# arnab39/equiadapt

Hardware: AMD Instinct MI355X
Metric: canonicalize+invert images/sec (224x224 C8) (higher is better)
Workload: dtype f32 (resampling / FFT / accumulation in fp32; the network's channel contraction as 2xfp16 split of every fp32 operand (within one fp32 ulp), 3 exact products, fp32 accumulate -- closer to fp64 than the fp32 matrix instruction, see step_ms_by_gemm_form); 1 GPU; configs[1]: 224x224x3 synthetic, C8, GroupEquivariantImageCanonicalization + ESCNNEquivariantNetwork in e2cnn's LAYER SHAPES (32 fields x 8 = 256 ch, k5, 3 layers, crop 0.8, resize 96) with this repository's own filter-bank parameterisation (bilinear-rotated banks; e2cnn's steerable basis is not restated -- e2cnn-trained weights enter via load_exported_dense), forward, then invert_canonicalization; batch_per_gpu=256, global_batch=256, parallelism=dp1 (no collective in the forward path)

## Files before the change

### equiadapt_amd/csrc/cgemm3m_bf16.hip

```cpp
#include "eqa_common.hpp"

#ifdef EQA_BLK_CLOCK
namespace {
__device__ long long g_blk_clock[16];
struct BlkClock {
  long long c0, w0, e0, t_epi;
  unsigned long long tk[8], tot[8];
  __device__ __forceinline__ BlkClock() : c0(clock64()), w0(wall_clock64()), e0(0), t_epi(0), tk{}, tot{} {}
  __device__ __forceinline__ void tick(int i) {
    if constexpr (EQA_BLK_CLOCK >= 2) {
      __builtin_amdgcn_sched_barrier(0);
      asm volatile("s_memtime %0" : "=s"(tk[i]));
    }
  }
  __device__ __forceinline__ void stage_end() {
    if constexpr (EQA_BLK_CLOCK >= 2) {
      tick(5);
      asm volatile("s_waitcnt lgkmcnt(0)" ::: "memory");
#pragma unroll
      for (int i = 0; i < 5; ++i) tot[i] += tk[i + 1] - tk[i];
    }
  }
  __device__ __forceinline__ void tile_epilogue_begin() { e0 = clock64(); }
  __device__ __forceinline__ void tile_epilogue_end() { t_epi += clock64() - e0; }
  __device__ __forceinline__ void publish() {
    if (blockIdx.x == 100 && threadIdx.x == 0) {
      g_blk_clock[0] = clock64() - c0; g_blk_clock[1] = wall_clock64() - w0; g_blk_clock[2] = t_epi;
      for (int i = 0; i < 7; ++i) g_blk_clock[3 + i] = (long long)tot[i];
    }
  }
};
}
extern "C" int eqa_debug_blk_clock(long long* out) { return (int)hipMemcpyFromSymbol(out, HIP_SYMBOL(g_blk_clock), 80); }
#else
namespace {
struct BlkClock {
  __device__ __forceinline__ void tick(int) {}
  __device__ __forceinline__ void stage_end() {}
  __device__ __forceinline__ void tile_epilogue_begin() {}
  __device__ __forceinline__ void tile_epilogue_end() {}
  __device__ __forceinline__ void publish() {}
};
}
#endif

namespace {

#include "cgemm3m_common.inc"

typedef __bf16 bf16x8 __attribute__((ext_vector_type(8)));
typedef unsigned u32x2 __attribute__((ext_vector_type(2)));

constexpr unsigned kHi = 0xffff0000u;

__device__ __forceinline__ void split3(const float a, unsigned (&x)[3]) {
  const float p1 = __builtin_bit_cast(float, __builtin_bit_cast(unsigned, a) & kHi);
  const float r1 = a - p1;
  const float p2 = __builtin_bit_cast(float, __builtin_bit_cast(unsigned, r1) & kHi);
  const float r2 = r1 - p2;
  x[0] = __builtin_bit_cast(unsigned, a);
  x[1] = __builtin_bit_cast(unsigned, r1);
  x[2] = __builtin_bit_cast(unsigned, r2);
}
__device__ __forceinline__ unsigned pack_hi(const unsigned lo, const unsigned hi) { return __builtin_amdgcn_perm(hi, lo, 0x07060302u); }

struct Pieces {
  u32x4 p[3];
};
__device__ __forceinline__ Pieces split8(const f32x4 lo, const f32x4 hi) {
  Pieces o;
  unsigned x[8][3];
#pragma unroll
  for (int e = 0; e < 8; ++e) split3(e < 4 ? lo[e & 3] : hi[e & 3], x[e]);
#pragma unroll
  for (int j = 0; j < 4; ++j)
#pragma unroll
    for (int q = 0; q < 3; ++q) o.p[q][j] = pack_hi(x[2 * j][q], x[2 * j + 1][q]);
  return o;
}
__device__ __forceinline__ void split4(const f32x4 v, u32x2 (&o)[3]) {
  unsigned x[4][3];
#pragma unroll
  for (int t = 0; t < 4; ++t) split3(v[t], x[t]);
#pragma unroll
  for (int q = 0; q < 3; ++q) {
    o[q][0] = pack_hi(x[0][q], x[1][q]);
    o[q][1] = pack_hi(x[2][q], x[3][q]);
  }
}

struct ARaw {
  f32x4 ar[2], ai[2];
};
struct BHalf {
  u32x4 b[3][3];
};
struct APieces {
  Pieces a[2][3];
};

constexpr unsigned kBFrag = 64 * 16;
constexpr unsigned kBTileBytes = 9 * kBFrag;

__device__ __forceinline__ void load_a(ARaw& o, const StageAddr& at, unsigned aoff) {
#pragma unroll
  for (int b = 0; b < 2; ++b) {
    o.ar[b] = buf_ld<f32x4>(at.a, aoff + 32 * b, at.sa);
    o.ai[b] = buf_ld<f32x4>(at.a, aoff + 32 * b + 64, at.sa);
  }
}
__device__ __forceinline__ void load_b(BHalf& o, const StageAddr& at, unsigned boff, int n) {
#pragma unroll
  for (int p = 0; p < 3; ++p)
#pragma unroll
    for (int q = 0; q < 3; ++q) o.b[p][q] = buf_ld<u32x4>(at.b, boff + ((n * 3 + p) * 3 + q) * kBFrag, at.sb);
}

__device__ __forceinline__ void split_a(APieces& P, const ARaw& r, int m) {
  P.a[m][0] = split8(r.ar[0], r.ar[1]);
  P.a[m][1] = split8(r.ai[0], r.ai[1]);
  P.a[m][2] = split8(r.ar[0] + r.ai[0], r.ar[1] + r.ai[1]);
}

__device__ __forceinline__ f32x16 mma(const u32x4 a, const u32x4 b, const f32x16 c) {
  return __builtin_amdgcn_mfma_f32_32x32x16_bf16(__builtin_bit_cast(bf16x8, a), __builtin_bit_cast(bf16x8, b), c, 0, 0, 0);
}

template <int TERMS>
__device__ __forceinline__ void mma_quarter(const APieces& P, const BHalf& B, f32x16 (&acc)[3][2][2], int m, int n) {
#pragma unroll
  for (int w = 0; w < 5; ++w)
#pragma unroll
    for (int pa = 0; pa < 3; ++pa) {
      const int pb = w - pa;
      if (pb < 0 || pb > 2 || (TERMS == 6 && w > 2)) continue;
#pragma unroll
      for (int p = 0; p < 3; ++p) acc[p][m][n] = mma(P.a[m][p].p[pa], B.b[p][pb], acc[p][m][n]);
    }
}

template <int NMMA, int NVALU, int NLOAD, int NSTORE, int NDS>
__device__ __forceinline__ void pin_quarter() {
  if (NDS) __builtin_amdgcn_sched_group_barrier(0x100, NDS, 0);
  constexpr int kMem = NLOAD + NSTORE;
  constexpr int kValuPer = (NVALU + NMMA - 1) / NMMA;
#pragma unroll
  for (int k = 0; k < NMMA; ++k) {
    __builtin_amdgcn_sched_group_barrier(0x008, 1, 0);
    if (k < NLOAD) __builtin_amdgcn_sched_group_barrier(0x020, 1, 0);
    else if (k < kMem) __builtin_amdgcn_sched_group_barrier(0x040, 1, 0);
    if (NVALU) __builtin_amdgcn_sched_group_barrier(0x002, kValuPer, 0);
  }
}

template <int NPAIR, int TERMS>
__device__ __forceinline__ void run_stage(APieces& P, ARaw& raw0, ARaw& raw1, BHalf& B0, BHalf& B1, f32x16 (&acc)[3][2][2],
                                          const StageAddr& cur, const StageAddr& nxt, unsigned naoff0, unsigned naoff1, unsigned boff,
                                          const float* lds_lane, const ParkedDst& dst, int p0) {
  constexpr int kQ = 3 * TERMS;
  constexpr int kSplit = 150;
  f32x4 park[NPAIR > 0 ? NPAIR : 1];
  __builtin_amdgcn_sched_barrier(0);
  load_b(B1, cur, boff, 1);
  load_a(raw0, nxt, naoff0);
  split_a(P, raw1, 1);
  mma_quarter<TERMS>(P, B0, acc, 0, 0);
  pin_quarter<kQ, kSplit, 13, 0, 0>();
  __builtin_amdgcn_sched_barrier(0);
  load_a(raw1, nxt, naoff1);
  mma_quarter<TERMS>(P, B0, acc, 1, 0);
  pin_quarter<kQ, 0, 4, 0, 0>();
  __builtin_amdgcn_sched_barrier(0);
#pragma unroll
  for (int k = 0; k < NPAIR; ++k) park[k] = *reinterpret_cast<const f32x4*>(lds_lane + (p0 + k) * (2 * kLdsRowFloats));
  load_b(B0, nxt, boff, 0);
  mma_quarter<TERMS>(P, B1, acc, 0, 1);
#pragma unroll
  for (int k = 0; k < NPAIR; ++k) store_pair(dst, p0 + k, park[k]);
  pin_quarter<kQ, 0, 9, NPAIR, NPAIR>();
  __builtin_amdgcn_sched_barrier(0);
  split_a(P, raw0, 0);
  mma_quarter<TERMS>(P, B1, acc, 1, 1);
  pin_quarter<kQ, kSplit, 0, 0, 0>();
  __builtin_amdgcn_sched_barrier(0);
}

template <int NPAIR, int TERMS>
__global__ __launch_bounds__(256, 1) void fft_cgemm3m_bf16_kernel(const float* __restrict__ V, const uint16_t* __restrict__ Bp,
                                                                  float* __restrict__ Mo, int M, int pitch, int Cin, int Cout, int F,
                                                                  int n_rt, int n_ct, int waves_per_xcd) {
  const int lane = threadIdx.x & 63;
  const int wave = __builtin_amdgcn_readfirstlane(threadIdx.x >> 6);
  const int xcd = blockIdx.x & (kXcd - 1);
  const int q = (blockIdx.x >> 3) * 4 + wave;
  const int S = Cin / kStageK;
  const int wpf = n_rt * n_ct;
  const int nf_x = (F - xcd + kXcd - 1) / kXcd;
  const int total = nf_x * wpf;
  if (q >= total) return;
  const int i = lane & 31, h = lane >> 5;
  __shared__ __attribute__((aligned(16))) float lds_all[4 * kLdsWaveFloats];
  float* lds_w = lds_all + wave * kLdsWaveFloats;
  const float* lds_lane = lds_w + h * kLdsRowFloats + i * 4;
  const WaveTileWalk<uint16_t, kBTileBytes> walk(V, Bp, Mo, M, pitch, Cin, Cout, xcd, wpf, n_ct, S, i, h);
  const unsigned boff = lane * 16;

  StageAddr at;
  unsigned aoff0, aoff1;
  int f, row0, ct;
  walk.locate(q, at, aoff0, aoff1, f, row0, ct);
  ParkedDst dst = walk.nothing_parked(f, row0, ct);
  ARaw raw0, raw1;
  APieces P;
  BHalf B0, B1;
  load_a(raw0, at, aoff0);
  load_a(raw1, at, aoff1);
  load_b(B0, at, boff, 0);
  split_a(P, raw0, 0);
  for (int u = q; u < total; u += waves_per_xcd) {
    f32x16 acc[3][2][2];
#pragma unroll
    for (int p = 0; p < 3; ++p)
#pragma unroll
      for (int m = 0; m < 2; ++m)
#pragma unroll
        for (int n = 0; n < 2; ++n)
#pragma unroll
          for (int e = 0; e < 16; ++e) acc[p][m][n][e] = 0.f;
    StageAddr nat;
    unsigned naoff0, naoff1;
    int nf, nrow0, nct;
    walk.locate(u + waves_per_xcd < total ? u + waves_per_xcd : u, nat, naoff0, naoff1, nf, nrow0, nct);
    for (int s = 0; s < S; ++s) {
      const bool more = s + 1 < S;
      if (NPAIR == 0) flush_rows(lds_lane, dst, (32 * s) / S, (32 * (s + 1)) / S);
      run_stage<NPAIR, TERMS>(P, raw0, raw1, B0, B1, acc, walk.at_stage(at, s), more ? walk.at_stage(at, s + 1) : nat,
                              more ? aoff0 : naoff0, more ? aoff1 : naoff1, boff, lds_lane, dst, s * NPAIR);
    }
    park_tile(acc, lds_w, i, h);
    dst = walk.parked(f, row0, ct);
    at = nat; aoff0 = naoff0; aoff1 = naoff1; f = nf; row0 = nrow0; ct = nct;
  }
  flush_rows(lds_lane, dst, 0, 32);
}

constexpr int kBlkM = 128, kBlkN = 128;
constexpr int kFragBytes = 64 * 16;
constexpr int kABufs = 3;
typedef _Float16 f16x8 __attribute__((ext_vector_type(8)));

constexpr int pieces_of(int terms) { return terms == 3 ? 2 : 3; }
constexpr int a_stage_bytes(int terms) { return 12 * pieces_of(terms) * kFragBytes; }

template <int NP>
struct BSet {
  u32x4 b[3][NP];
};
struct AFrags {
  u32x4 a[3];
};
struct RawA {
  f32x4 re[2], im[2];
};
struct TileAt {
  __amdgpu_buffer_rsrc_t a, b;
  unsigned sb;
};

typedef _Float16 f16x2v __attribute__((ext_vector_type(2)));
__device__ __forceinline__ void split4h(const f32x4 v, u32x2 (&o)[2]) {
#pragma unroll
  for (int j = 0; j < 2; ++j) {
    const float a = v[2 * j], b = v[2 * j + 1];
    const f16x2v h = {(_Float16)a, (_Float16)b};
    const f16x2v l = {(_Float16)(a - (float)h[0]), (_Float16)(b - (float)h[1])};
    o[0][j] = __builtin_bit_cast(unsigned, h);
    o[1][j] = __builtin_bit_cast(unsigned, l);
  }
}
template <int NP, int ROW, int PART>
__device__ __forceinline__ void split_part(const RawA& r, unsigned char* wr, const float scale) {
  const f32x4 v = PART == 0 ? r.re[ROW] : PART == 1 ? r.im[ROW] : r.re[ROW] + r.im[ROW];
  u32x2 o[NP];
  if constexpr (NP == 3) split4(v, o);
  else split4h(v * scale, o);
#pragma unroll
  for (int q = 0; q < NP; ++q) *reinterpret_cast<u32x2*>(wr + (ROW * 6 * NP + PART * NP + q) * kFragBytes) = o[q];
}
template <int ROW>
__device__ __forceinline__ void load_raw(RawA& o, const TileAt& t, unsigned voff, unsigned row64, unsigned soff) {
  o.re[ROW] = buf_ld<f32x4>(t.a, voff + ROW * row64, soff);
  o.im[ROW] = buf_ld<f32x4>(t.a, voff + ROW * row64 + 64, soff);
}
template <int NP>
__device__ __forceinline__ void load_bset(BSet<NP>& o, const TileAt& t, unsigned voff, unsigned soff) {
#pragma unroll
  for (int k = 0; k < 3 * NP; ++k) o.b[k / NP][k % NP] = buf_ld<u32x4>(t.b, voff + k * kBFrag, t.sb + soff);
}
template <int NP, int M, int PA>
__device__ __forceinline__ void read_frags(AFrags& o, const unsigned char* rd) {
#pragma unroll
  for (int p = 0; p < 3; ++p) o.a[p] = *reinterpret_cast<const u32x4*>(rd + ((M * 3 + p) * NP + PA) * kFragBytes);
}
template <int TERMS>
__device__ __forceinline__ f32x16 mma_t(const u32x4 a, const u32x4 b, const f32x16 c) {
  if constexpr (TERMS == 3) return __builtin_amdgcn_mfma_f32_32x32x16_f16(__builtin_bit_cast(f16x8, a), __builtin_bit_cast(f16x8, b), c, 0, 0, 0);
  else return mma(a, b, c);
}
template <int TERMS, int M, int PA, bool FIRST>
__device__ __forceinline__ void mma_rows(const AFrags& A, const BSet<pieces_of(TERMS)>& B, f32x16 (&acc)[3][4]) {
  const f32x16 zero = {0.f, 0.f, 0.f, 0.f, 0.f, 0.f, 0.f, 0.f, 0.f, 0.f, 0.f, 0.f, 0.f, 0.f, 0.f, 0.f};
#pragma unroll
  for (int pb = 0; pb < pieces_of(TERMS); ++pb) {
    if ((TERMS == 6 && PA + pb > 2) || (TERMS == 3 && PA + pb > 1)) continue;
#pragma unroll
    for (int p = 0; p < 3; ++p) acc[p][M] = mma_t<TERMS>(A.a[p], B.b[p][pb], FIRST && PA == 0 && pb == 0 ? zero : acc[p][M]);
  }
}
template <int NMMA, int NDSR, int NLOAD, int NVALU, int NDSW>
__device__ __forceinline__ void pin_region() {
  constexpr int kValuPer = (NVALU + NMMA - 1) / NMMA;
#pragma unroll
  for (int k = 0; k < NMMA; ++k) {
    __builtin_amdgcn_sched_group_barrier(0x008, 1, 0);
    if (k < NDSR) __builtin_amdgcn_sched_group_barrier(0x100, 1, 0);
    if (k < NLOAD) __builtin_amdgcn_sched_group_barrier(0x020, 1, 0);
    if (NVALU) __builtin_amdgcn_sched_group_barrier(0x002, kValuPer, 0);
    if (k >= NMMA - NDSW) __builtin_amdgcn_sched_group_barrier(0x200, 1, 0);
  }
}

template <int TERMS, bool FIRST>
__device__ __forceinline__ void run_stage_block(const BSet<pieces_of(TERMS)>& Bc, BSet<pieces_of(TERMS)>& Bn, RawA& raw, AFrags& F0,
                                                AFrags& F1, AFrags& F2, AFrags& F3,
                                                f32x16 (&acc)[3][4], const unsigned char* rd, const unsigned char* rd_next,
                                                unsigned char* wr, const TileAt& tb, unsigned sb_off, unsigned b_voff, const TileAt& ta,
                                                unsigned sa_off, unsigned a_voff, unsigned row64, const float scale, BlkClock& clk) {
  constexpr int NP = pieces_of(TERMS);
  constexpr int kN = TERMS == 9 ? 27 : TERMS == 6 ? 18 : 9;
  constexpr int kSplit = NP == 3 ? 32 : 20;
  constexpr int kRd = 3 * NP;
  clk.tick(0);
  __builtin_amdgcn_sched_barrier(0);
  read_frags<NP, 0, 1>(F1, rd);
  if constexpr (NP == 3) read_frags<NP, 0, 2>(F2, rd);
  read_frags<NP, 1, 0>(F3, rd);
  load_bset<NP>(Bn, tb, b_voff, sb_off);
  split_part<NP, 0, 0>(raw, wr, scale);
  mma_rows<TERMS, 0, 0, FIRST>(F0, Bc, acc); mma_rows<TERMS, 0, 1, FIRST>(F1, Bc, acc);
  if constexpr (NP == 3) mma_rows<TERMS, 0, 2, FIRST>(F2, Bc, acc);
  pin_region<kN, kRd, kRd, kSplit, NP>();
  clk.tick(1);
  __builtin_amdgcn_sched_barrier(0);
  read_frags<NP, 1, 1>(F1, rd);
  if constexpr (NP == 3) read_frags<NP, 1, 2>(F2, rd);
  read_frags<NP, 2, 0>(F0, rd);
  split_part<NP, 0, 1>(raw, wr, scale); split_part<NP, 0, 2>(raw, wr, scale);
  mma_rows<TERMS, 1, 0, FIRST>(F3, Bc, acc); mma_rows<TERMS, 1, 1, FIRST>(F1, Bc, acc);
  if constexpr (NP == 3) mma_rows<TERMS, 1, 2, FIRST>(F2, Bc, acc);
  pin_region<kN, kRd, 0, 2 * kSplit + 4, 2 * NP>();
  clk.tick(2);
  __builtin_amdgcn_sched_barrier(0);
  read_frags<NP, 2, 1>(F1, rd);
  if constexpr (NP == 3) read_frags<NP, 2, 2>(F2, rd);
  read_frags<NP, 3, 0>(F3, rd);
  split_part<NP, 1, 0>(raw, wr, scale); split_part<NP, 1, 1>(raw, wr, scale);
  mma_rows<TERMS, 2, 0, FIRST>(F0, Bc, acc); mma_rows<TERMS, 2, 1, FIRST>(F1, Bc, acc);
  if constexpr (NP == 3) mma_rows<TERMS, 2, 2, FIRST>(F2, Bc, acc);
  pin_region<kN, kRd, 0, 2 * kSplit, 2 * NP>();
  clk.tick(3);
  __builtin_amdgcn_sched_barrier(0);
  read_frags<NP, 3, 1>(F1, rd);
  if constexpr (NP == 3) read_frags<NP, 3, 2>(F2, rd);
  read_frags<NP, 0, 0>(F0, rd_next);
  split_part<NP, 1, 2>(raw, wr, scale);
  load_raw<0>(raw, ta, a_voff, row64, sa_off);
  mma_rows<TERMS, 3, 0, FIRST>(F3, Bc, acc); mma_rows<TERMS, 3, 1, FIRST>(F1, Bc, acc);
  if constexpr (NP == 3) mma_rows<TERMS, 3, 2, FIRST>(F2, Bc, acc);
  pin_region<kN, kRd, 2, kSplit + 4, NP>();
  __builtin_amdgcn_sched_barrier(0);
  load_raw<1>(raw, ta, a_voff, row64, sa_off);
  clk.tick(4);
  __builtin_amdgcn_sched_barrier(0);
  asm volatile("s_waitcnt lgkmcnt(0)\n\ts_barrier" ::: "memory");
  clk.stage_end();
}

template <int TERMS>
__global__ __launch_bounds__(256, 1) void fft_cgemm3m_bf16_block_kernel(const float* __restrict__ V, const uint16_t* __restrict__ Bp,
                                                                        float* __restrict__ Mo, int M, int pitch, int Cin, int Cout, int F,
                                                                        int n_rt, int n_cg, int blocks_per_xcd,
                                                                        const float* __restrict__ vbound, int nbound, float b_scale) {
  constexpr int NP = pieces_of(TERMS);
  constexpr int kAStageBytes = a_stage_bytes(TERMS);
  const int lane = threadIdx.x & 63;
  const int wave = __builtin_amdgcn_readfirstlane(threadIdx.x >> 6);
  const int xcd = blockIdx.x & (kXcd - 1);
  const int q = blockIdx.x >> 3;
  const int S = Cin / kStageK;
  const int tpf = n_rt * n_cg;
  const int nf_x = (F - xcd + kXcd - 1) / kXcd;
  const int total = nf_x * tpf;
  if (q >= total) return;
  BlkClock clk;
  extern __shared__ __attribute__((aligned(16))) unsigned char lds[];
  const size_t rowf = (size_t)2 * Cin, mo_row = (size_t)2 * Cout;
  const unsigned b_stage_bytes = (unsigned)(Cout / 32) * 3 * NP * kBFrag;
  const unsigned a_stage = 32u * 4u;
  const unsigned b_voff = lane * 16;
  const unsigned row64 = (unsigned)(64 * rowf * 4);
  const int sp_b = lane & 1, sp_r = (lane >> 1) & 15, sp_h = lane >> 5;
  const int sp_row = 16 * wave + sp_r;
  const unsigned sp_lds = (unsigned)((sp_row >> 5) * 3 * NP * kFragBytes + ((sp_row & 31) + 32 * sp_h) * 16 + 8 * sp_b);
  const unsigned sp_k = (unsigned)(8 * sp_b + 4 * sp_h) * 4u;

  auto locate = [&](int u, TileAt& at, unsigned& aoff, int& f, int& row0, int& ct) {
    const bool live = u < total;
    const int uu = live ? u : 0;
    const int fi = uu / tpf, r = uu - fi * tpf;
    f = xcd + kXcd * fi;
    const int rt = r / n_cg, cg = r - rt * n_cg;
    row0 = rt * kBlkM;
    ct = 4 * cg + wave;
    at.a = __builtin_amdgcn_make_buffer_rsrc(const_cast<float*>(V) + (size_t)f * pitch * rowf, 0, live ? (unsigned)((size_t)pitch * rowf * 4) : 0u, 0x00020000);
    aoff = (unsigned)((size_t)(row0 + sp_row) * rowf * 4) + sp_k;
    at.b = __builtin_amdgcn_make_buffer_rsrc(const_cast<uint16_t*>(Bp) + (size_t)f * S * (b_stage_bytes / 2), 0, live ? (unsigned)S * b_stage_bytes : 0u, 0x00020000);
    at.sb = (unsigned)ct * (3 * NP * kBFrag);
  };

  TileAt ta, tb;
  unsigned a_voff, b_unused;
  int ua = q, sa = 0, ub = q, sb = 0;
  int fa, rowa, cta, f, row0, ct;
  locate(q, ta, a_voff, f, row0, ct);
  tb = ta;
  auto next_a = [&]() {
    if (++sa == S) { sa = 0; ua += blocks_per_xcd; locate(ua, ta, a_voff, fa, rowa, cta); }
  };
  auto next_b = [&]() {
    if (++sb == S) { sb = 0; ub += blocks_per_xcd; locate(ub, tb, b_unused, fa, rowa, cta); }
  };

  float a_scale = 1.0f, out_scale = 1.0f;
  if constexpr (TERMS == 3) {
    float mx = 0.0f;
    for (int t = lane; t < nbound; t += 64) mx = fmaxf(mx, vbound[t]);
#pragma unroll
    for (int o = 32; o > 0; o >>= 1) mx = fmaxf(mx, __shfl_xor(mx, o));
    int ex = 0;
    if (mx > 0.0f && mx < 3.0e38f) (void)frexpf(mx, &ex);
    ex = min(max(14 - ex, -100), 100);
    ex = __builtin_amdgcn_readfirstlane(ex);
    a_scale = ldexpf(1.0f, ex);
    out_scale = ldexpf(1.0f, -ex) / b_scale;
  }
  RawA raw0, raw1;
  BSet<NP> B0, B1;
  AFrags F0, F1, F2, F3;
  load_raw<0>(raw0, ta, a_voff, row64, sa * a_stage); load_raw<1>(raw0, ta, a_voff, row64, sa * a_stage); next_a();
  load_raw<0>(raw1, ta, a_voff, row64, sa * a_stage); load_raw<1>(raw1, ta, a_voff, row64, sa * a_stage); next_a();
  load_bset<NP>(B0, tb, b_voff, sb * b_stage_bytes); next_b();
  {
    unsigned char* w0p = lds + sp_lds;
    unsigned char* w1p = lds + kAStageBytes + sp_lds;
    split_part<NP, 0, 0>(raw0, w0p, a_scale); split_part<NP, 0, 1>(raw0, w0p, a_scale); split_part<NP, 0, 2>(raw0, w0p, a_scale);
    split_part<NP, 1, 0>(raw0, w0p, a_scale); split_part<NP, 1, 1>(raw0, w0p, a_scale); split_part<NP, 1, 2>(raw0, w0p, a_scale);
    split_part<NP, 0, 0>(raw1, w1p, a_scale); split_part<NP, 0, 1>(raw1, w1p, a_scale); split_part<NP, 0, 2>(raw1, w1p, a_scale);
    split_part<NP, 1, 0>(raw1, w1p, a_scale); split_part<NP, 1, 1>(raw1, w1p, a_scale); split_part<NP, 1, 2>(raw1, w1p, a_scale);
  }
  load_raw<0>(raw0, ta, a_voff, row64, sa * a_stage); load_raw<1>(raw0, ta, a_voff, row64, sa * a_stage); next_a();
  load_raw<0>(raw1, ta, a_voff, row64, sa * a_stage); load_raw<1>(raw1, ta, a_voff, row64, sa * a_stage); next_a();
  asm volatile("s_waitcnt lgkmcnt(0)\n\ts_barrier" ::: "memory");
  unsigned rbuf = 0;
  read_frags<NP, 0, 0>(F0, lds + lane * 16);
  auto step = [&](unsigned o) { return o + kAStageBytes >= kABufs * kAStageBytes ? o + kAStageBytes - kABufs * kAStageBytes : o + kAStageBytes; };

  for (int u = q; u < total; u += blocks_per_xcd) {
    f32x16 acc[3][4];
#define EQA_STAGE(FIRST, BC, BN, RAW)                                                                                                 \
  {                                                                                                                                  \
    const unsigned r1 = step(rbuf), r2 = step(r1);                                                                                   \
    run_stage_block<TERMS, FIRST>(BC, BN, RAW, F0, F1, F2, F3, acc, lds + rbuf + lane * 16, lds + r1 + lane * 16, lds + r2 + sp_lds, \
                                  tb, sb * b_stage_bytes, b_voff, ta, sa * a_stage, a_voff, row64, a_scale, clk);                            \
    next_a(); next_b();                                                                                                              \
    rbuf = r1;                                                                                                                       \
  }
    EQA_STAGE(true, B0, B1, raw0)
    EQA_STAGE(false, B1, B0, raw1)
    for (int s = 2; s < S; s += 2) {
      EQA_STAGE(false, B0, B1, raw0)
      EQA_STAGE(false, B1, B0, raw1)
    }
#undef EQA_STAGE
    clk.tile_epilogue_begin();
    {
      const int rows = __builtin_amdgcn_readfirstlane(min(kBlkM, M - row0));
      const __amdgpu_buffer_rsrc_t dr =
          __builtin_amdgcn_make_buffer_rsrc(Mo + ((size_t)f * pitch + row0) * mo_row, 0, (unsigned)(rows * mo_row * 4), 0x00020000);
      const int i = lane & 31, h = lane >> 5;
      const unsigned voff = (unsigned)((4 * h * mo_row + (size_t)(32 * ct + i) * 2) * 4);
#pragma unroll
      for (int m = 0; m < 4; ++m)
#pragma unroll
        for (int e = 0; e < 16; ++e) {
          const unsigned roff = voff + (unsigned)((32 * m + (e & 3) + 8 * (e >> 2)) * mo_row * 4);
          const float t1 = acc[0][m][e], t2 = acc[1][m][e], t3 = acc[2][m][e];
          u32x2 c;
          c[0] = __builtin_bit_cast(unsigned, TERMS == 3 ? (t1 - t2) * out_scale : t1 - t2);
          c[1] = __builtin_bit_cast(unsigned, TERMS == 3 ? (t3 - t1 - t2) * out_scale : t3 - t1 - t2);
          __builtin_amdgcn_raw_buffer_store_b64(c, dr, roff, 0, 0);
        }
    }
    int nf, nrow0, nct;
    TileAt unused_t;
    unsigned unused_o;
    locate(u + blocks_per_xcd, unused_t, unused_o, nf, nrow0, nct);
    f = nf; row0 = nrow0; ct = nct;
    clk.tile_epilogue_end();
  }
  clk.publish();
}

__global__ __launch_bounds__(256) void spectra3m_split_kernel(const float* __restrict__ B3, uint16_t* __restrict__ Bp, size_t groups) {
  const size_t t = (size_t)blockIdx.x * blockDim.x + threadIdx.x;
  if (t >= groups * 64) return;
  const size_t g = t >> 6;
  const int lane = (int)(t & 63);
  const float* src = B3 + g * (2 * 64 * 4) + lane * 4;
  const f32x4 lo = *reinterpret_cast<const f32x4*>(src), hi = *reinterpret_cast<const f32x4*>(src + 64 * 4);
  const Pieces p = split8(lo, hi);
  u32x4* dst = reinterpret_cast<u32x4*>(Bp + g * (3 * 64 * 8)) + lane;
#pragma unroll
  for (int q = 0; q < 3; ++q) dst[q * 64] = p.p[q];
}


__global__ __launch_bounds__(256) void spectra3m_split_f16_kernel(const float* __restrict__ B3, uint16_t* __restrict__ Bh, size_t groups,
                                                                  float b_scale) {
  const size_t t = (size_t)blockIdx.x * blockDim.x + threadIdx.x;
  if (t >= groups * 64) return;
  const size_t g = t >> 6;
  const int lane = (int)(t & 63);
  const float* src = B3 + g * (2 * 64 * 4) + lane * 4;
  const f32x4 lo = *reinterpret_cast<const f32x4*>(src) * b_scale, hi = *reinterpret_cast<const f32x4*>(src + 64 * 4) * b_scale;
  u32x2 a[2], b[2];
  split4h(lo, a);
  split4h(hi, b);
  u32x4* dst = reinterpret_cast<u32x4*>(Bh + g * (2 * 64 * 8)) + lane;
#pragma unroll
  for (int q = 0; q < 2; ++q) {
    const u32x4 v = {a[q][0], a[q][1], b[q][0], b[q][1]};
    dst[q * 64] = v;
  }
}

template <int TERMS>
int launch_block(const float* V, const void* B, float* Mo, int64_t M, int Cin, int Cout, const float* vbound, int nbound, float b_scale,
                 void* stream) {
  const int n_rb = (int)((M + kBlkM - 1) / kBlkM), n_cg = Cout / kBlkN;
  constexpr int kLds = kABufs * a_stage_bytes(TERMS);
  if (!allow_dynamic_lds((const void*)fft_cgemm3m_bf16_block_kernel<TERMS>, kLds)) return EQA_ERR_LAUNCH;
  hipLaunchKernelGGL((fft_cgemm3m_bf16_block_kernel<TERMS>), dim3(kGridBlocks), dim3(256), kLds, (hipStream_t)stream, V,
                     static_cast<const uint16_t*>(B), Mo, (int)M, (int)eqa_fft48k5_tile_pitch(M), Cin, Cout, eqa_fft48k5_frequencies(), n_rb,
                     n_cg, kBlocksPerXcd, vbound, nbound, b_scale);
  return launch_status();
}

}

namespace eqa {
int g_cgemm_bf16_form = 0;
}

extern "C" {

int64_t eqa_fft48k5_spectra3m_bf16_bytes(int Cin, int Cout) {
  if (!eqa_fft48k5_cgemm3m_supported(Cin, Cout)) return 0;
  return (int64_t)eqa_fft48k5_frequencies() * Cin * Cout * 3 * 3 * 2;
}

int eqa_fft48k5_spectra3m_split(const float* B3, void* Bp, int Cin, int Cout, void* stream) {
  if (!B3 || !Bp) return EQA_ERR_INVALID_ARG;
  if (!eqa_fft48k5_cgemm3m_supported(Cin, Cout) || (((uintptr_t)B3 | (uintptr_t)Bp) & 15)) return EQA_ERR_UNSUPPORTED;
  const size_t groups = (size_t)eqa_fft48k5_frequencies() * (Cin / kStageK) * (Cout / 32) * 3;
  const size_t threads = groups * 64;
  hipLaunchKernelGGL(spectra3m_split_kernel, dim3((unsigned)((threads + 255) / 256)), dim3(256), 0, (hipStream_t)stream, B3,
                     static_cast<uint16_t*>(Bp), groups);
  return launch_status();
}

int eqa_fft48k5_cgemm3m_bf16x3(const float* V, const void* Bp, float* Mo, int64_t M, int Cin, int Cout, int terms, void* stream) {
  if (terms != 9 && terms != 6) return EQA_ERR_INVALID_ARG;
  const int st = check_contraction_args(V, Bp, Mo, M, Cin, Cout);
  if (st != EQA_OK) return st == kNothingToDo ? EQA_OK : st;
  if ((int64_t)Cin * Cout * 9 * 2 > 0x7fffffffLL) return EQA_ERR_UNSUPPORTED;
  if (Cout % kBlkN == 0 && eqa::g_cgemm_bf16_form != 1) {
    return terms == 9 ? launch_block<9>(V, Bp, Mo, M, Cin, Cout, nullptr, 0, 1.0f, stream)
                      : launch_block<6>(V, Bp, Mo, M, Cin, Cout, nullptr, 0, 1.0f, stream);
  }
  const int F = eqa_fft48k5_frequencies();
  const int n_rt = (int)((M + kTileM - 1) / kTileM), n_ct = Cout / kTileN;
  const int S = Cin / kStageK;
#define EQA_CG_LAUNCH(NP, T)                                                                                                            \
  hipLaunchKernelGGL((fft_cgemm3m_bf16_kernel<NP, T>), dim3(kGridBlocks), dim3(256), 0, (hipStream_t)stream, V,                         \
                     static_cast<const uint16_t*>(Bp), Mo, (int)M, (int)eqa_fft48k5_tile_pitch(M), Cin, Cout, F, n_rt, n_ct, kWavesPerXcd)
#define EQA_CG_TERMS(NP) do { if (terms == 9) EQA_CG_LAUNCH(NP, 9); else EQA_CG_LAUNCH(NP, 6); } while (0)
  switch (32 % S == 0 ? 32 / S : 0) {
    case 4: EQA_CG_TERMS(4); break;
    case 2: EQA_CG_TERMS(2); break;
    case 1: EQA_CG_TERMS(1); break;
    default: EQA_CG_TERMS(0); break;
  }
#undef EQA_CG_TERMS
#undef EQA_CG_LAUNCH
  return launch_status();
}


int64_t eqa_fft48k5_spectra3m_f16_bytes(int Cin, int Cout) {
  if (!eqa_fft48k5_cgemm3m_supported(Cin, Cout) || Cout % kBlkN != 0) return 0;
  return (int64_t)eqa_fft48k5_frequencies() * Cin * Cout * 3 * 2 * 2;
}

int eqa_fft48k5_spectra3m_split_f16(const float* B3, void* Bh, int Cin, int Cout, float b_scale, void* stream) {
  if (!B3 || !Bh || !(b_scale > 0.0f)) return EQA_ERR_INVALID_ARG;
  if (eqa_fft48k5_spectra3m_f16_bytes(Cin, Cout) == 0 || (((uintptr_t)B3 | (uintptr_t)Bh) & 15)) return EQA_ERR_UNSUPPORTED;
  int ex = 0;
  if (frexpf(b_scale, &ex) != 0.5f) return EQA_ERR_INVALID_ARG;
  const size_t groups = (size_t)eqa_fft48k5_frequencies() * (Cin / kStageK) * (Cout / 32) * 3;
  const size_t threads = groups * 64;
  hipLaunchKernelGGL(spectra3m_split_f16_kernel, dim3((unsigned)((threads + 255) / 256)), dim3(256), 0, (hipStream_t)stream, B3,
                     static_cast<uint16_t*>(Bh), groups, b_scale);
  return launch_status();
}

int eqa_fft48k5_cgemm3m_f16x2(const float* V, const void* Bh, float* Mo, int64_t M, int Cin, int Cout, const float* vbound, int nbound,
                              float b_scale, void* stream) {
  if (!vbound || nbound <= 0 || !(b_scale > 0.0f)) return EQA_ERR_INVALID_ARG;
  const int st = check_contraction_args(V, Bh, Mo, M, Cin, Cout);
  if (st != EQA_OK) return st == kNothingToDo ? EQA_OK : st;
  if (Cout % kBlkN != 0 || (Cin / kStageK) % 2 != 0 || (int64_t)Cin * Cout * 6 * 2 > 0x7fffffffLL) return EQA_ERR_UNSUPPORTED;
  return launch_block<3>(V, Bh, Mo, M, Cin, Cout, vbound, nbound, b_scale, stream);
}

}
```

Before: 74840 images/s.

## Overlap tile epilogue stores with last K-stage matrix instructions

The final K-stage of each tile becomes a specialized LAST variant. Once an accumulator row block is final, its output stores are interleaved with the remaining matrix instructions of later row blocks, so only the last row block is written in the separate epilogue. This hides the serial store epilogue behind MFMA work. Stores also get a nontemporal cache hint, and the timing probe gains a last-stage counter. The cost is more complex scheduling pins and a restructured stage loop, which may disturb register pressure or instruction ordering.

```diff
diff --git a/equiadapt_amd/csrc/cgemm3m_bf16.hip b/equiadapt_amd/csrc/cgemm3m_bf16.hip
--- a/equiadapt_amd/csrc/cgemm3m_bf16.hip
+++ b/equiadapt_amd/csrc/cgemm3m_bf16.hip
@@ -4,9 +4,9 @@
 namespace {
 __device__ long long g_blk_clock[16];
 struct BlkClock {
-  long long c0, w0, e0, t_epi;
+  long long c0, w0, e0, t_epi, l0, t_last;
   unsigned long long tk[8], tot[8];
-  __device__ __forceinline__ BlkClock() : c0(clock64()), w0(wall_clock64()), e0(0), t_epi(0), tk{}, tot{} {}
+  __device__ __forceinline__ BlkClock() : c0(clock64()), w0(wall_clock64()), e0(0), t_epi(0), l0(0), t_last(0), tk{}, tot{} {}
   __device__ __forceinline__ void tick(int i) {
     if constexpr (EQA_BLK_CLOCK >= 2) {
       __builtin_amdgcn_sched_barrier(0);
@@ -21,12 +21,15 @@
       for (int i = 0; i < 5; ++i) tot[i] += tk[i + 1] - tk[i];
     }
   }
+  __device__ __forceinline__ void last_stage_begin() { l0 = clock64(); }
+  __device__ __forceinline__ void last_stage_end() { t_last += clock64() - l0; }
   __device__ __forceinline__ void tile_epilogue_begin() { e0 = clock64(); }
   __device__ __forceinline__ void tile_epilogue_end() { t_epi += clock64() - e0; }
   __device__ __forceinline__ void publish() {
     if (blockIdx.x == 100 && threadIdx.x == 0) {
       g_blk_clock[0] = clock64() - c0; g_blk_clock[1] = wall_clock64() - w0; g_blk_clock[2] = t_epi;
-      for (int i = 0; i < 7; ++i) g_blk_clock[3 + i] = (long long)tot[i];
+      for (int i = 0; i < 6; ++i) g_blk_clock[3 + i] = (long long)tot[i];
+      g_blk_clock[9] = t_last;
     }
   }
 };
@@ -37,6 +40,8 @@
 struct BlkClock {
   __device__ __forceinline__ void tick(int) {}
   __device__ __forceinline__ void stage_end() {}
+  __device__ __forceinline__ void last_stage_begin() {}
+  __device__ __forceinline__ void last_stage_end() {}
   __device__ __forceinline__ void tile_epilogue_begin() {}
   __device__ __forceinline__ void tile_epilogue_end() {}
   __device__ __forceinline__ void publish() {}
@@ -329,13 +334,101 @@
     if (k >= NMMA - NDSW) __builtin_amdgcn_sched_group_barrier(0x200, 1, 0);
   }
 }
-
-template <int TERMS, bool FIRST>
+template <int NMMA, int NDSR, int NLOAD, int NVALU, int NDSW>
+__device__ __forceinline__ void pin_region_head() {
+  constexpr int kValuPer = (NVALU + NMMA - 1) / NMMA, kRdPer = (NDSR + NMMA - 1) / NMMA;
+#pragma unroll
+  for (int k = 0; k < NMMA; ++k) {
+    __builtin_amdgcn_sched_group_barrier(0x008, 1, 0);
+    __builtin_amdgcn_sched_group_barrier(0x100, kRdPer, 0);
+    if (k < NLOAD) __builtin_amdgcn_sched_group_barrier(0x020, 1, 0);
+    __builtin_amdgcn_sched_group_barrier(0x002, kValuPer, 0);
+  }
+  __builtin_amdgcn_sched_group_barrier(0x200, NDSW, 0);
+}
+
+struct TileDst {
+  __amdgpu_buffer_rsrc_t dr;
+  unsigned voff, row_bytes;
+  float out_scale;
+};
+constexpr int kStoreNt = 2;
+template <int TERMS, int MQ, int E0 = 0, int E1 = 16>
+__device__ __forceinline__ void retire_rows(const f32x16 (&acc)[3][4], const TileDst& d) {
+#pragma unroll
+  for (int e = E0; e < E1; ++e) {
+    const unsigned roff = d.voff + (unsigned)(32 * MQ + (e & 3) + 8 * (e >> 2)) * d.row_bytes;
+    const float t1 = acc[0][MQ][e], t2 = acc[1][MQ][e], t3 = acc[2][MQ][e];
+    u32x2 c;
+    c[0] = __builtin_bit_cast(unsigned, TERMS == 3 ? (t1 - t2) * d.out_scale : t1 - t2);
+    c[1] = __builtin_bit_cast(unsigned, TERMS == 3 ? (t3 - t1 - t2) * d.out_scale : t3 - t1 - t2);
+    __builtin_amdgcn_raw_buffer_store_b64(c, d.dr, roff, 0, kStoreNt);
+  }
+}
+
+template <int TERMS>
+constexpr int mma_code(int k) {
+  int n = 0;
+  for (int pa = 0; pa < pieces_of(TERMS); ++pa)
+    for (int pb = 0; pb < pieces_of(TERMS); ++pb) {
+      if ((TERMS == 6 && pa + pb > 2) || (TERMS == 3 && pa + pb > 1)) continue;
+      for (int p = 0; p < 3; ++p)
+        if (n++ == k) return (pa * 3 + pb) * 3 + p;
+    }
+  return -1;
+}
+template <int TERMS, int M, int K>
+__device__ __forceinline__ void mma_one(const AFrags& Fa, const AFrags& Fb, const AFrags& Fc, const BSet<pieces_of(TERMS)>& B,
+                                        f32x16 (&acc)[3][4]) {
+  constexpr int code = mma_code<TERMS>(K), pa = code / 9, pb = code / 3 % 3, p = code % 3;
+  static_assert(code >= 0, "no such matrix instruction in a region");
+  const AFrags& A = pa == 0 ? Fa : pa == 1 ? Fb : Fc;
+  acc[p][M] = mma_t<TERMS>(A.a[p], B.b[p][pb], acc[p][M]);
+}
+template <int TERMS, int M, int K>
+__device__ __forceinline__ void retire_slot(const AFrags& Fa, const AFrags& Fb, const AFrags& Fc, const BSet<pieces_of(TERMS)>& B,
+                                            f32x16 (&acc)[3][4], const TileDst& d) {
+  constexpr int kN = 3 * (TERMS == 3 ? 3 : TERMS), kS = kN / 3, kR = kN - kS;
+  constexpr int kRet = TERMS == 3 ? 9 : 7;
+  constexpr int e0 = (K - kS) * 16 / kR, e1 = (K - kS + 1) * 16 / kR;
+  mma_one<TERMS, M, K>(Fa, Fb, Fc, B, acc);
+  retire_rows<TERMS, M - 1, e0, e1>(acc, d);
+  __builtin_amdgcn_sched_group_barrier(0x008, 1, 0);
+#pragma unroll
+  for (int e = e0; e < e1; ++e) {
+    __builtin_amdgcn_sched_group_barrier(0x002, kRet, 0);
+    __builtin_amdgcn_sched_group_barrier(0x040, 1, 0);
+  }
+  __builtin_amdgcn_sched_barrier(0);
+}
+template <int TERMS, int M, int K0, int... K>
+__device__ __forceinline__ void retire_slots(const AFrags& Fa, const AFrags& Fb, const AFrags& Fc, const BSet<pieces_of(TERMS)>& B,
+                                             f32x16 (&acc)[3][4], const TileDst& d, std::integer_sequence<int, K...>) {
+  (retire_slot<TERMS, M, K0 + K>(Fa, Fb, Fc, B, acc, d), ...);
+}
+template <int TERMS, int M, int... K>
+__device__ __forceinline__ void mma_head(const AFrags& Fa, const AFrags& Fb, const AFrags& Fc, const BSet<pieces_of(TERMS)>& B,
+                                         f32x16 (&acc)[3][4], std::integer_sequence<int, K...>) {
+  (mma_one<TERMS, M, K>(Fa, Fb, Fc, B, acc), ...);
+}
+template <int TERMS, int M, int NLOAD, int NVALU, int NDSW>
+__device__ __forceinline__ void run_retire_region(const AFrags& Fa, const AFrags& Fb, const AFrags& Fc,
+                                                  const BSet<pieces_of(TERMS)>& B, f32x16 (&acc)[3][4], const TileDst& d) {
+  constexpr int kN = 3 * (TERMS == 3 ? 3 : TERMS), kS = kN / 3;
+  mma_head<TERMS, M>(Fa, Fb, Fc, B, acc, std::make_integer_sequence<int, kS>{});
+  pin_region_head<kS, 3 * pieces_of(TERMS), NLOAD, NVALU, NDSW>();
+  __builtin_amdgcn_sched_barrier(0);
+  retire_slots<TERMS, M, kS>(Fa, Fb, Fc, B, acc, d, std::make_integer_sequence<int, kN - kS>{});
+}
+
+template <int TERMS, bool FIRST, bool LAST>
 __device__ __forceinline__ void run_stage_block(const BSet<pieces_of(TERMS)>& Bc, BSet<pieces_of(TERMS)>& Bn, RawA& raw, AFrags& F0,
                                                 AFrags& F1, AFrags& F2, AFrags& F3,
                                                 f32x16 (&acc)[3][4], const unsigned char* rd, const unsigned char* rd_next,
                                                 unsigned char* wr, const TileAt& tb, unsigned sb_off, unsigned b_voff, const TileAt& ta,
-                                                unsigned sa_off, unsigned a_voff, unsigned row64, const float scale, BlkClock& clk) {
+                                                unsigned sa_off, unsigned a_voff, unsigned row64, const float scale, const TileDst& dst,
+                                                BlkClock& clk) {
+  static_assert(!(FIRST && LAST), "a tile has two K-stages at least");
   constexpr int NP = pieces_of(TERMS);
   constexpr int kN = TERMS == 9 ? 27 : TERMS == 6 ? 18 : 9;
   constexpr int kSplit = NP == 3 ? 32 : 20;
@@ -356,18 +449,26 @@
   if constexpr (NP == 3) read_frags<NP, 1, 2>(F2, rd);
   read_frags<NP, 2, 0>(F0, rd);
   split_part<NP, 0, 1>(raw, wr, scale); split_part<NP, 0, 2>(raw, wr, scale);
-  mma_rows<TERMS, 1, 0, FIRST>(F3, Bc, acc); mma_rows<TERMS, 1, 1, FIRST>(F1, Bc, acc);
-  if constexpr (NP == 3) mma_rows<TERMS, 1, 2, FIRST>(F2, Bc, acc);
-  pin_region<kN, kRd, 0, 2 * kSplit + 4, 2 * NP>();
+  if constexpr (LAST) {
+    run_retire_region<TERMS, 1, 0, 2 * kSplit + 4, 2 * NP>(F3, F1, F2, Bc, acc, dst);
+  } else {
+    mma_rows<TERMS, 1, 0, FIRST>(F3, Bc, acc); mma_rows<TERMS, 1, 1, FIRST>(F1, Bc, acc);
+    if constexpr (NP == 3) mma_rows<TERMS, 1, 2, FIRST>(F2, Bc, acc);
+    pin_region<kN, kRd, 0, 2 * kSplit + 4, 2 * NP>();
+  }
   clk.tick(2);
   __builtin_amdgcn_sched_barrier(0);
   read_frags<NP, 2, 1>(F1, rd);
   if constexpr (NP == 3) read_frags<NP, 2, 2>(F2, rd);
   read_frags<NP, 3, 0>(F3, rd);
   split_part<NP, 1, 0>(raw, wr, scale); split_part<NP, 1, 1>(raw, wr, scale);
-  mma_rows<TERMS, 2, 0, FIRST>(F0, Bc, acc); mma_rows<TERMS, 2, 1, FIRST>(F1, Bc, acc);
-  if constexpr (NP == 3) mma_rows<TERMS, 2, 2, FIRST>(F2, Bc, acc);
-  pin_region<kN, kRd, 0, 2 * kSplit, 2 * NP>();
+  if constexpr (LAST) {
+    run_retire_region<TERMS, 2, 0, 2 * kSplit, 2 * NP>(F0, F1, F2, Bc, acc, dst);
+  } else {
+    mma_rows<TERMS, 2, 0, FIRST>(F0, Bc, acc); mma_rows<TERMS, 2, 1, FIRST>(F1, Bc, acc);
+    if constexpr (NP == 3) mma_rows<TERMS, 2, 2, FIRST>(F2, Bc, acc);
+    pin_region<kN, kRd, 0, 2 * kSplit, 2 * NP>();
+  }
   clk.tick(3);
   __builtin_amdgcn_sched_barrier(0);
   read_frags<NP, 3, 1>(F1, rd);
@@ -375,9 +476,13 @@
   read_frags<NP, 0, 0>(F0, rd_next);
   split_part<NP, 1, 2>(raw, wr, scale);
   load_raw<0>(raw, ta, a_voff, row64, sa_off);
-  mma_rows<TERMS, 3, 0, FIRST>(F3, Bc, acc); mma_rows<TERMS, 3, 1, FIRST>(F1, Bc, acc);
-  if constexpr (NP == 3) mma_rows<TERMS, 3, 2, FIRST>(F2, Bc, acc);
-  pin_region<kN, kRd, 2, kSplit + 4, NP>();
+  if constexpr (LAST) {
+    run_retire_region<TERMS, 3, 2, kSplit + 4, NP>(F3, F1, F2, Bc, acc, dst);
+  } else {
+    mma_rows<TERMS, 3, 0, FIRST>(F3, Bc, acc); mma_rows<TERMS, 3, 1, FIRST>(F1, Bc, acc);
+    if constexpr (NP == 3) mma_rows<TERMS, 3, 2, FIRST>(F2, Bc, acc);
+    pin_region<kN, kRd, 2, kSplit + 4, NP>();
+  }
   __builtin_amdgcn_sched_barrier(0);
   load_raw<1>(raw, ta, a_voff, row64, sa_off);
   clk.tick(4);
@@ -477,40 +582,35 @@
 
   for (int u = q; u < total; u += blocks_per_xcd) {
     f32x16 acc[3][4];
-#define EQA_STAGE(FIRST, BC, BN, RAW)                                                                                                 \
+    TileDst dst;
+#define EQA_STAGE(FIRST, LAST, BC, BN, RAW)                                                                                           \
   {                                                                                                                                  \
     const unsigned r1 = step(rbuf), r2 = step(r1);                                                                                   \
-    run_stage_block<TERMS, FIRST>(BC, BN, RAW, F0, F1, F2, F3, acc, lds + rbuf + lane * 16, lds + r1 + lane * 16, lds + r2 + sp_lds, \
-                                  tb, sb * b_stage_bytes, b_voff, ta, sa * a_stage, a_voff, row64, a_scale, clk);                            \
+    run_stage_block<TERMS, FIRST, LAST>(BC, BN, RAW, F0, F1, F2, F3, acc, lds + rbuf + lane * 16, lds + r1 + lane * 16,              \
+                                        lds + r2 + sp_lds, tb, sb * b_stage_bytes, b_voff, ta, sa * a_stage, a_voff, row64, a_scale,  \
+                                        dst, clk);                                                                                   \
     next_a(); next_b();                                                                                                              \
     rbuf = r1;                                                                                                                       \
   }
-    EQA_STAGE(true, B0, B1, raw0)
-    EQA_STAGE(false, B1, B0, raw1)
+    EQA_STAGE(true, false, B0, B1, raw0)
     for (int s = 2; s < S; s += 2) {
-      EQA_STAGE(false, B0, B1, raw0)
-      EQA_STAGE(false, B1, B0, raw1)
+      EQA_STAGE(false, false, B1, B0, raw1)
+      EQA_STAGE(false, false, B0, B1, raw0)
     }
+    {
+      const int rows = __builtin_amdgcn_readfirstlane(min(kBlkM, M - row0));
+      dst.dr = __builtin_amdgcn_make_buffer_rsrc(Mo + ((size_t)f * pitch + row0) * mo_row, 0, (unsigned)(rows * mo_row * 4), 0x00020000);
+      const int i = lane & 31, h = lane >> 5;
+      dst.voff = (unsigned)((4 * h * mo_row + (size_t)(32 * ct + i) * 2) * 4);
+      dst.row_bytes = (unsigned)(mo_row * 4);
+      dst.out_scale = out_scale;
+    }
+    clk.last_stage_begin();
+    EQA_STAGE(false, true, B1, B0, raw1)
+    clk.last_stage_end();
 #undef EQA_STAGE
     clk.tile_epilogue_begin();
-    {
-      const int rows = __builtin_amdgcn_readfirstlane(min(kBlkM, M - row0));
-      const __amdgpu_buffer_rsrc_t dr =
-          __builtin_amdgcn_make_buffer_rsrc(Mo + ((size_t)f * pitch + row0) * mo_row, 0, (unsigned)(rows * mo_row * 4), 0x00020000);
-      const int i = lane & 31, h = lane >> 5;
-      const unsigned voff = (unsigned)((4 * h * mo_row + (size_t)(32 * ct + i) * 2) * 4);
-#pragma unroll
-      for (int m = 0; m < 4; ++m)
-#pragma unroll
-        for (int e = 0; e < 16; ++e) {
-          const unsigned roff = voff + (unsigned)((32 * m + (e & 3) + 8 * (e >> 2)) * mo_row * 4);
-          const float t1 = acc[0][m][e], t2 = acc[1][m][e], t3 = acc[2][m][e];
-          u32x2 c;
-          c[0] = __builtin_bit_cast(unsigned, TERMS == 3 ? (t1 - t2) * out_scale : t1 - t2);
-          c[1] = __builtin_bit_cast(unsigned, TERMS == 3 ? (t3 - t1 - t2) * out_scale : t3 - t1 - t2);
-          __builtin_amdgcn_raw_buffer_store_b64(c, dr, roff, 0, 0);
-        }
-    }
+    retire_rows<TERMS, 3>(acc, dst);
     int nf, nrow0, nct;
     TileAt unused_t;
     unsigned unused_o;
```

New measurement: 75040 images/s, median of 6. Within noise of the previous version (+0.3%).
